# Visual-Behavior/aloception-oss

Measured on AMD Instinct MI355X. Metric: frames/sec (whole node) DeformableDETR-R50 inference, higher is better.
Workload: dtype bf16; 1 GPU; DeformableDETR-R50 inference bf16, batch 8 synthetic 1333x800 frames per GPU, random-init weights; launch=hip-graph replay + eager inference(), per_gpu_batch=8, global_batch=8, parallelism=batch-sharded x1, no collective

## Files before the change

aloception-oss_amd/csrc/gemm.hip:

```cpp
#include "common.hpp"

namespace alo {
namespace {

constexpr int kRows = 64;
constexpr int kOutStride = 64 * 2 + 16;

typedef __attribute__((ext_vector_type(8))) __bf16 bf16x8_t;

__device__ __forceinline__ bf16x8_t as_bf16x8(const u32x4& v) {
    union { u32x4 u; bf16x8_t b; } x;
    x.u = v;
    return x.b;
}

struct GemmDims {
    long M;
    int N;
    int tiles;
    int S;
    int gs, gWo, gHoWo, gW, gHW;
};

template <typename D>
__device__ __forceinline__ long gather_row(const D& dm, long row) {
    if (dm.gs <= 1) return row;
    const long n = row / dm.gHoWo;
    const int rem = (int)(row - n * dm.gHoWo);
    const int yo = rem / dm.gWo, xo = rem - yo * dm.gWo;
    return n * dm.gHW + (long)(yo * dm.gs) * dm.gW + xo * dm.gs;
}

template <int kK, bool RELU, bool HAS_RES, bool HM>
__global__ void __launch_bounds__(256, 2)
linear_shortk_kernel(const bf16_t* __restrict__ X, const bf16_t* __restrict__ W, const bf16_t* __restrict__ bias,
                     const bf16_t* __restrict__ R, bf16_t* __restrict__ Y, const GemmDims dm) {
    constexpr int kRowBytes = kK * 2 + 16;
    constexpr int kSteps = kK / 16;
    constexpr int kPieces = kK / 8;
    constexpr int kLoads = kRows * kPieces / 256;
    static_assert(kRows * kPieces % 256 == 0, "the tile loader gives every thread the same number of pieces");
    extern __shared__ __attribute__((aligned(16))) unsigned char smem[];
    unsigned char* const xbuf = smem;
    const int tid = threadIdx.x, wave = tid >> 6, lane = tid & 63;
    unsigned char* obuf = smem + kRows * kRowBytes + wave * (kRows * kOutStride);

    const int col0 = blockIdx.y * 256 + wave * 64;
    const bool has_cols = col0 < dm.N;
    const int nl = lane & 31, kg = lane >> 5;

    u32x4 wreg[2][kSteps];
    float* const bias_tab = reinterpret_cast<float*>(smem + kRows * kRowBytes + 4 * (kRows * kOutStride)) + wave * 64;
    if (has_cols) {
#pragma unroll
        for (int t = 0; t < 2; ++t) {
            const bf16_t* wr = W + (size_t)(col0 + 32 * t + nl) * kK + 8 * kg;
#pragma unroll
            for (int s = 0; s < kSteps; ++s) wreg[t][s] = *reinterpret_cast<const u32x4*>(wr + 16 * s);
        }
        const int r = lane & 15, t = (lane >> 4) & 1, k2 = lane >> 5;
        bias_tab[lane] = bias != nullptr ? bf16_to_f32(bias[col0 + 32 * t + (r & 3) + 8 * (r >> 2) + 4 * k2].bits) : 0.f;
    }

    auto fetch = [&](int tile, u32x4 (&r)[kLoads]) {
#pragma unroll
        for (int j = 0; j < kLoads; ++j) {
            const int p = tid + 256 * j;
            long row = (long)tile * kRows + p / kPieces;
            row = gather_row(dm, row < dm.M ? row : dm.M - 1);
            r[j] = *reinterpret_cast<const u32x4*>(X + row * kK + (p % kPieces) * 8);
        }
    };
    auto park = [&](const u32x4 (&r)[kLoads]) {
#pragma unroll
        for (int j = 0; j < kLoads; ++j) {
            const int p = tid + 256 * j;
            *reinterpret_cast<u32x4*>(xbuf + (p / kPieces) * kRowBytes + (p % kPieces) * 16) = r[j];
        }
    };

    int tile = blockIdx.x;
    if (tile >= dm.tiles) return;
    u32x4 stage[kLoads];
    fetch(tile, stage);

    for (;;) {
        park(stage);
        __syncthreads();
        const int next = tile + gridDim.x;
        const bool more = next < dm.tiles;
        if (more) fetch(next, stage);

        if (has_cols) {
#pragma unroll
            for (int half = 0; half < kRows / 32; ++half) {
                f32x16 acc[2];
#pragma unroll
                for (int t = 0; t < 2; ++t)
#pragma unroll
                    for (int q = 0; q < 4; ++q) {
                        const f32x4 b4 = *reinterpret_cast<const f32x4*>(bias_tab + (kg * 2 + t) * 16 + 4 * q);
#pragma unroll
                        for (int i = 0; i < 4; ++i) acc[t][4 * q + i] = b4[i];
                    }
#pragma unroll
                for (int s = 0; s < kSteps; ++s) {
                    const u32x4 a = *reinterpret_cast<const u32x4*>(xbuf + (32 * half + nl) * kRowBytes + (16 * s + 8 * kg) * 2);
                    acc[0] = __builtin_amdgcn_mfma_f32_32x32x16_bf16(as_bf16x8(wreg[0][s]), as_bf16x8(a), acc[0], 0, 0, 0);
                    acc[1] = __builtin_amdgcn_mfma_f32_32x32x16_bf16(as_bf16x8(wreg[1][s]), as_bf16x8(a), acc[1], 0, 0, 0);
                }
#pragma unroll
                for (int t = 0; t < 2; ++t)
#pragma unroll
                    for (int q = 0; q < 4; ++q) {
                        float v0 = acc[t][4 * q], v1 = acc[t][4 * q + 1], v2 = acc[t][4 * q + 2], v3 = acc[t][4 * q + 3];
                        if (RELU && !HAS_RES) { v0 = relu_keep_nan(v0); v1 = relu_keep_nan(v1); v2 = relu_keep_nan(v2); v3 = relu_keep_nan(v3); }
                        *reinterpret_cast<u32x2*>(obuf + (32 * half + nl) * kOutStride + (32 * t + 8 * q + 4 * kg) * 2) =
                            u32x2{pack_bf16x2(v0, v1), pack_bf16x2(v2, v3)};
                    }
            }
            __builtin_amdgcn_fence(__ATOMIC_RELEASE, "wavefront");
            __builtin_amdgcn_wave_barrier();
            __builtin_amdgcn_fence(__ATOMIC_ACQUIRE, "wavefront");
            if constexpr (HM) {
                const unsigned char* mask = reinterpret_cast<const unsigned char*>(R);
                const int heads = dm.N / 32;
#pragma unroll
                for (int hh = 0; hh < 2; ++hh) {
#pragma unroll
                    for (int pass = 0; pass < kRows / 16; ++pass) {
                        const int row = pass * 16 + (lane >> 2);
                        const long grow = (long)tile * kRows + row;
                        if (grow < dm.M) {
                            u32x4 v = *reinterpret_cast<const u32x4*>(obuf + row * kOutStride + hh * 64 + (lane & 3) * 16);
                            if (mask != nullptr && mask[grow]) v = u32x4{0u, 0u, 0u, 0u};
                            const long nb = grow / dm.S, sp = grow - nb * dm.S;
                            const int head = col0 / 32 + hh;
                            *reinterpret_cast<u32x4*>(Y + ((nb * heads + head) * dm.S + sp) * 32 + (lane & 3) * 8) = v;
                        }
                    }
                }
            } else
#pragma unroll
            for (int pass = 0; pass < kRows / 8; ++pass) {
                const int row = pass * 8 + (lane >> 3);
                const long grow = (long)tile * kRows + row;
                u32x4 v = *reinterpret_cast<const u32x4*>(obuf + row * kOutStride + (lane & 7) * 16);
                if (grow < dm.M) {
                    if constexpr (HAS_RES) {
                        const u32x4 rv = *reinterpret_cast<const u32x4*>(R + grow * dm.N + col0 + (lane & 7) * 8);
                        const unsigned a4[4] = {v.x, v.y, v.z, v.w}, r4[4] = {rv.x, rv.y, rv.z, rv.w};
                        unsigned o4[4];
#pragma unroll
                        for (int i = 0; i < 4; ++i) {
                            float lo = __uint_as_float(a4[i] << 16) + __uint_as_float(r4[i] << 16);
                            float hi = __uint_as_float(a4[i] & 0xffff0000u) + __uint_as_float(r4[i] & 0xffff0000u);
                            if (RELU) { lo = relu_keep_nan(lo); hi = relu_keep_nan(hi); }
                            o4[i] = pack_bf16x2(lo, hi);
                        }
                        v = u32x4{o4[0], o4[1], o4[2], o4[3]};
                    }
                    *reinterpret_cast<u32x4*>(Y + grow * dm.N + col0 + (lane & 7) * 8) = v;
                }
            }
        }
        if (!more) break;
        __syncthreads();
        tile = next;
    }
}

}
}

using namespace alo;

namespace {
template <int K, bool RELU, bool HAS_RES, bool HM = false>
int launch_shortk(const void* x, const void* weight, const void* bias, const void* residual, void* y, long M, int N,
                  hipStream_t stream, int S = 0, const int* gather = nullptr) {
    GemmDims dm;
    dm.M = M; dm.N = N; dm.tiles = (int)((M + kRows - 1) / kRows); dm.S = S;
    dm.gs = gather ? gather[0] : 1;
    dm.gWo = gather ? gather[2] : 1; dm.gHoWo = gather ? gather[1] * gather[2] : 1;
    dm.gW = gather ? gather[4] : 1; dm.gHW = gather ? gather[3] * gather[4] : 1;
    const size_t lds = kRows * (K * 2 + 16) + 4 * kRows * kOutStride + 4 * 64 * sizeof(float);
    const int cols = (N + 255) / 256;
    int gx = 512 / cols;
    if (gx > dm.tiles) gx = dm.tiles;
    if (gx < 1) gx = 1;
    void* args[] = {&x, &weight, &bias, &residual, &y, &dm};
    static unsigned long long attr_done = 0;
    (void)ensure_dynamic_lds(reinterpret_cast<const void*>(linear_shortk_kernel<K, RELU, HAS_RES, HM>), (int)lds, &attr_done);
    hipError_t e = hipLaunchKernel(reinterpret_cast<const void*>(linear_shortk_kernel<K, RELU, HAS_RES, HM>), dim3(gx, cols), dim3(256), args,
                                   lds, stream);
    if (e != hipSuccess) return fail(ALO_ERR_LAUNCH, "alo_linear_shortk: %s", hipGetErrorString(e));
    return check_launch("alo_linear_shortk");
}
}

extern "C" int alo_linear_shortk(const void* x, const void* weight, const void* bias, const void* residual, void* y, long M,
                                 int N, int K, int relu, int dtype, void* stream) {
    ALO_REQUIRE(x && weight && y, ALO_ERR_INVALID_ARGUMENT, "alo_linear_shortk: null pointer argument");
    ALO_REQUIRE(M > 0 && N > 0 && N % 64 == 0, ALO_ERR_INVALID_ARGUMENT,
                "alo_linear_shortk: M must be positive and N a positive multiple of 64 (M=%ld N=%d)", M, N);
    ALO_REQUIRE(K == 64 || K == 128 || K == 256, ALO_ERR_UNSUPPORTED, "alo_linear_shortk: K must be 64, 128 or 256, got %d", K);
    ALO_REQUIRE(dtype == ALO_BF16, ALO_ERR_UNSUPPORTED, "alo_linear_shortk: bf16 only (dtype %d)", dtype);
    ALO_REQUIRE((((uintptr_t)x | (uintptr_t)weight | (uintptr_t)y | (uintptr_t)residual) & 15) == 0, ALO_ERR_INVALID_ARGUMENT,
                "alo_linear_shortk: pointers must be 16-byte aligned");
    hipStream_t st = static_cast<hipStream_t>(stream);
#define ALO_GEMM_CASE(KK)                                                                                       \
    if (K == KK) {                                                                                               \
        if (residual) return relu ? launch_shortk<KK, true, true>(x, weight, bias, residual, y, M, N, st)       \
                                  : launch_shortk<KK, false, true>(x, weight, bias, residual, y, M, N, st);     \
        return relu ? launch_shortk<KK, true, false>(x, weight, bias, residual, y, M, N, st)                    \
                    : launch_shortk<KK, false, false>(x, weight, bias, residual, y, M, N, st);                  \
    }
    ALO_GEMM_CASE(64) ALO_GEMM_CASE(128) ALO_GEMM_CASE(256)
#undef ALO_GEMM_CASE
    return ALO_ERR_UNSUPPORTED;
}

extern "C" int alo_internal_shortk_gather(const void* x, const void* weight, const void* bias, const void* residual, void* y,
                                          long M, int N, int K, int relu, const int* gather, void* stream) {
    hipStream_t st = static_cast<hipStream_t>(stream);
#define ALO_GEMM_CASE(KK)                                                                                                  \
    if (K == KK) {                                                                                                          \
        if (residual) return relu ? launch_shortk<KK, true, true>(x, weight, bias, residual, y, M, N, st, 0, gather)       \
                                  : launch_shortk<KK, false, true>(x, weight, bias, residual, y, M, N, st, 0, gather);     \
        return relu ? launch_shortk<KK, true, false>(x, weight, bias, residual, y, M, N, st, 0, gather)                    \
                    : launch_shortk<KK, false, false>(x, weight, bias, residual, y, M, N, st, 0, gather);                  \
    }
    ALO_GEMM_CASE(64) ALO_GEMM_CASE(128) ALO_GEMM_CASE(256)
#undef ALO_GEMM_CASE
    return fail(ALO_ERR_UNSUPPORTED, "alo_conv1x1_nhwc: the resident-weight kernel needs Cin in (64, 128, 256), got %d", K);
}

namespace alo {
namespace {

constexpr int kFfnRows = 64;
constexpr int kFfnStride = 256 * 2 + 16;

struct FfnDims {
    long M;
    int F;
    int tiles;
};

__global__ void __launch_bounds__(256, 2)
ffn256_kernel(const bf16_t* __restrict__ X, const bf16_t* __restrict__ W1, const bf16_t* __restrict__ B1,
              const bf16_t* __restrict__ W2, const bf16_t* __restrict__ B2, bf16_t* __restrict__ Y, const FfnDims dm) {
    extern __shared__ __attribute__((aligned(16))) unsigned char smem[];
    unsigned char* const xs = smem;
    unsigned char* const hs = smem + kFfnRows * kFfnStride;
    const int tid = threadIdx.x, wave = tid >> 6, lane = tid & 63;
    const int nl = lane & 31, kg = lane >> 5;
    const int F = dm.F;

    float* const b1s = reinterpret_cast<float*>(smem + 2 * kFfnRows * kFfnStride);
    float* const b2s = b1s + F;
    for (int i = tid; i < F; i += 256) b1s[i] = B1 ? bf16_to_f32(B1[i].bits) : 0.f;
    b2s[tid] = B2 ? bf16_to_f32(B2[tid].bits) : 0.f;

    constexpr int KB = 2;
    constexpr int NBATCH = 16 / KB;
    auto load_batch = [&](u32x4 (&buf)[2][KB], const bf16_t* frag0, size_t tile_stride, int batch) {
#pragma unroll
        for (int t = 0; t < 2; ++t)
#pragma unroll
            for (int j = 0; j < KB; ++j)
                buf[t][j] = *reinterpret_cast<const u32x4*>(frag0 + t * tile_stride + (size_t)(KB * batch + j) * 512);
        __builtin_amdgcn_sched_barrier(0);
    };
    auto mma_batch = [&](f32x16 (&acc)[2][2], const unsigned char* a_lds, const u32x4 (&buf)[2][KB], int batch) {
        u32x4 af[2][KB];
#pragma unroll
        for (int j = 0; j < KB; ++j) {
            const int s = KB * batch + j;
            af[0][j] = *reinterpret_cast<const u32x4*>(a_lds + nl * kFfnStride + (16 * s + 8 * kg) * 2);
            af[1][j] = *reinterpret_cast<const u32x4*>(a_lds + (32 + nl) * kFfnStride + (16 * s + 8 * kg) * 2);
        }
#pragma unroll
        for (int j = 0; j < KB; ++j) {
            const u32x4 a0 = af[0][j], a1 = af[1][j];
            acc[0][0] = __builtin_amdgcn_mfma_f32_32x32x16_bf16(as_bf16x8(buf[0][j]), as_bf16x8(a0), acc[0][0], 0, 0, 0);
            acc[0][1] = __builtin_amdgcn_mfma_f32_32x32x16_bf16(as_bf16x8(buf[1][j]), as_bf16x8(a0), acc[0][1], 0, 0, 0);
            acc[1][0] = __builtin_amdgcn_mfma_f32_32x32x16_bf16(as_bf16x8(buf[0][j]), as_bf16x8(a1), acc[1][0], 0, 0, 0);
            acc[1][1] = __builtin_amdgcn_mfma_f32_32x32x16_bf16(as_bf16x8(buf[1][j]), as_bf16x8(a1), acc[1][1], 0, 0, 0);
        }
        __builtin_amdgcn_sched_barrier(0);
    };
    const int fs = F / 16;
    auto w1_frag = [&](int r0) { return W1 + ((size_t)((r0 + 64 * wave) / 32) * 16 * 64 + lane) * 8; };
    auto w2_frag = [&](int r0) { return W2 + (((size_t)(2 * wave) * fs + r0 / 16) * 64 + lane) * 8; };

    for (int tile = blockIdx.x; tile < dm.tiles; tile += gridDim.x) {
        {
            u32x4 xv[8];
#pragma unroll
            for (int j = 0; j < 8; ++j) {
                const int p = tid + 256 * j;
                long row = (long)tile * kFfnRows + (p >> 5);
                row = row < dm.M ? row : dm.M - 1;
                xv[j] = *reinterpret_cast<const u32x4*>(X + row * 256 + (p & 31) * 8);
            }
#pragma unroll
            for (int j = 0; j < 8; ++j) {
                const int p = tid + 256 * j;
                *reinterpret_cast<u32x4*>(xs + (p >> 5) * kFfnStride + (p & 31) * 16) = xv[j];
            }
        }
        u32x4 bufa[2][KB], bufb[2][KB];
        load_batch(bufa, w1_frag(0), (size_t)16 * 512, 0);
        __syncthreads();

        f32x16 acc2[2][2];
#pragma unroll
        for (int a = 0; a < 2; ++a)
#pragma unroll
            for (int t = 0; t < 2; ++t)
#pragma unroll
                for (int i = 0; i < 16; ++i) acc2[a][t][i] = 0.f;

        for (int r0 = 0; r0 < F; r0 += 256) {
            f32x16 acc1[2][2];
#pragma unroll
            for (int a = 0; a < 2; ++a)
#pragma unroll
                for (int t = 0; t < 2; ++t)
#pragma unroll
                    for (int i = 0; i < 16; ++i) acc1[a][t][i] = 0.f;
            const bf16_t* w1p = w1_frag(r0);
            const bf16_t* w2p = w2_frag(r0);
#pragma unroll
            for (int bt = 0; bt < NBATCH; bt += 2) {
                load_batch(bufb, w1p, (size_t)16 * 512, bt + 1);
                mma_batch(acc1, xs, bufa, bt);
                if (bt + 2 < NBATCH) load_batch(bufa, w1p, (size_t)16 * 512, bt + 2);
                else load_batch(bufa, w2p, (size_t)fs * 512, 0);
                mma_batch(acc1, xs, bufb, bt + 1);
            }
#pragma unroll
            for (int t = 0; t < 2; ++t)
#pragma unroll
                for (int q = 0; q < 4; ++q) {
                    const int col = 64 * wave + 32 * t + 8 * q + 4 * kg;
                    const f32x4 bb = *reinterpret_cast<const f32x4*>(b1s + r0 + col);
#pragma unroll
                    for (int a = 0; a < 2; ++a) {
                        const float v0 = relu_keep_nan(acc1[a][t][4 * q] + bb[0]), v1 = relu_keep_nan(acc1[a][t][4 * q + 1] + bb[1]);
                        const float v2 = relu_keep_nan(acc1[a][t][4 * q + 2] + bb[2]), v3 = relu_keep_nan(acc1[a][t][4 * q + 3] + bb[3]);
                        *reinterpret_cast<u32x2*>(hs + (32 * a + nl) * kFfnStride + col * 2) = u32x2{pack_bf16x2(v0, v1), pack_bf16x2(v2, v3)};
                    }
                }
            __syncthreads();

#pragma unroll
            for (int bt = 0; bt < NBATCH; bt += 2) {
                load_batch(bufb, w2p, (size_t)fs * 512, bt + 1);
                mma_batch(acc2, hs, bufa, bt);
                if (bt + 2 < NBATCH) load_batch(bufa, w2p, (size_t)fs * 512, bt + 2);
                else if (r0 + 256 < F) load_batch(bufa, w1_frag(r0 + 256), (size_t)16 * 512, 0);
                mma_batch(acc2, hs, bufb, bt + 1);
            }
            __syncthreads();
        }

#pragma unroll
        for (int t = 0; t < 2; ++t)
#pragma unroll
            for (int q = 0; q < 4; ++q) {
                const int col = 64 * wave + 32 * t + 8 * q + 4 * kg;
                const f32x4 bb = *reinterpret_cast<const f32x4*>(b2s + col);
#pragma unroll
                for (int a = 0; a < 2; ++a)
                    *reinterpret_cast<u32x2*>(hs + (32 * a + nl) * kFfnStride + col * 2) =
                        u32x2{pack_bf16x2(acc2[a][t][4 * q] + bb[0], acc2[a][t][4 * q + 1] + bb[1]),
                              pack_bf16x2(acc2[a][t][4 * q + 2] + bb[2], acc2[a][t][4 * q + 3] + bb[3])};
            }
        __syncthreads();
#pragma unroll
        for (int j = 0; j < 8; ++j) {
            const int p = tid + 256 * j;
            const long row = (long)tile * kFfnRows + (p >> 5);
            if (row < dm.M)
                *reinterpret_cast<u32x4*>(Y + row * 256 + (p & 31) * 8) =
                    *reinterpret_cast<const u32x4*>(hs + (p >> 5) * kFfnStride + (p & 31) * 16);
        }
        __syncthreads();
    }
}

}
}

namespace alo {
namespace {
__global__ void __launch_bounds__(256)
pack_mfma_b_kernel(const bf16_t* __restrict__ W, bf16_t* __restrict__ P, int N, int K) {
    const long total = (long)N * K / 8;
    for (long i = (long)blockIdx.x * 256 + threadIdx.x; i < total; i += (long)gridDim.x * 256) {
        const int lane = (int)(i % 64);
        const long frag = i / 64;
        const int s = (int)(frag % (K / 16)), t = (int)(frag / (K / 16));
        const int n = 32 * t + (lane & 31), k = 16 * s + 8 * (lane >> 5);
        *reinterpret_cast<u32x4*>(P + i * 8) = *reinterpret_cast<const u32x4*>(W + (size_t)n * K + k);
    }
}
}
}

extern "C" int alo_pack_mfma_b(const void* w, void* packed, int N, int K, int dtype, void* stream) {
    ALO_REQUIRE(w && packed, ALO_ERR_INVALID_ARGUMENT, "alo_pack_mfma_b: null pointer argument");
    ALO_REQUIRE(N > 0 && K > 0 && N % 32 == 0 && K % 16 == 0, ALO_ERR_INVALID_ARGUMENT,
                "alo_pack_mfma_b: N must be a multiple of 32 and K a multiple of 16 (N=%d K=%d)", N, K);
    ALO_REQUIRE(dtype == ALO_BF16, ALO_ERR_UNSUPPORTED, "alo_pack_mfma_b: bf16 only (dtype %d)", dtype);
    long total = (long)N * K / 8;
    unsigned blocks = (unsigned)((total + 255) / 256 > 4096 ? 4096 : (total + 255) / 256);
    void* args[] = {&w, &packed, &N, &K};
    hipError_t e = hipLaunchKernel(reinterpret_cast<const void*>(pack_mfma_b_kernel), dim3(blocks), dim3(256), args, 0,
                                   static_cast<hipStream_t>(stream));
    if (e != hipSuccess) return fail(ALO_ERR_LAUNCH, "alo_pack_mfma_b: %s", hipGetErrorString(e));
    return check_launch("alo_pack_mfma_b");
}

extern "C" int alo_ffn256(const void* x, const void* w1, const void* b1, const void* w2, const void* b2, void* y, long M,
                          int F, int dtype, void* stream) {
    ALO_REQUIRE(x && w1 && w2 && y, ALO_ERR_INVALID_ARGUMENT, "alo_ffn256: null pointer argument");
    ALO_REQUIRE(M > 0 && F > 0 && F % 256 == 0, ALO_ERR_INVALID_ARGUMENT,
                "alo_ffn256: M must be positive and the hidden width a positive multiple of 256 (M=%ld F=%d)", M, F);
    ALO_REQUIRE(dtype == ALO_BF16, ALO_ERR_UNSUPPORTED, "alo_ffn256: bf16 only (dtype %d)", dtype);
    ALO_REQUIRE((((uintptr_t)x | (uintptr_t)w1 | (uintptr_t)w2 | (uintptr_t)y) & 15) == 0, ALO_ERR_INVALID_ARGUMENT,
                "alo_ffn256: pointers must be 16-byte aligned");
    FfnDims dm;
    dm.M = M; dm.F = F; dm.tiles = (int)((M + kFfnRows - 1) / kFfnRows);
    const size_t lds = 2 * kFfnRows * kFfnStride + ((size_t)F + 256) * sizeof(float);
    int gx = dm.tiles < 512 ? dm.tiles : 512;
    void* args[] = {&x, &w1, &b1, &w2, &b2, &y, &dm};
    if (lds > 160 * 1024) return fail(ALO_ERR_UNSUPPORTED, "alo_ffn256: hidden width %d needs %zu bytes of LDS", F, lds);
    {
        static int limit_set[64] = {0};
        int dev = 0;
        (void)hipGetDevice(&dev);
        if ((int)lds > __atomic_load_n(&limit_set[dev & 63], __ATOMIC_ACQUIRE)) {
            if (hipFuncSetAttribute(reinterpret_cast<const void*>(ffn256_kernel), hipFuncAttributeMaxDynamicSharedMemorySize, (int)lds) == hipSuccess)
                __atomic_store_n(&limit_set[dev & 63], (int)lds, __ATOMIC_RELEASE);
        }
    }
    hipError_t e = hipLaunchKernel(reinterpret_cast<const void*>(ffn256_kernel), dim3(gx), dim3(256), args, lds,
                                   static_cast<hipStream_t>(stream));
    if (e != hipSuccess) return fail(ALO_ERR_LAUNCH, "alo_ffn256: %s", hipGetErrorString(e));
    return check_launch("alo_ffn256");
}

extern "C" int alo_value_proj_head_major(const void* x, const void* weight, const void* bias, const void* padding_mask,
                                         void* value_hm, int batch, int S, int heads, int K, int dtype, void* stream) {
    ALO_REQUIRE(x && weight && value_hm, ALO_ERR_INVALID_ARGUMENT, "alo_value_proj_head_major: null pointer argument");
    ALO_REQUIRE(batch > 0 && S > 0 && heads > 0 && heads % 2 == 0, ALO_ERR_INVALID_ARGUMENT,
                "alo_value_proj_head_major: batch, S must be positive and the head count even (batch=%d S=%d heads=%d)", batch, S,
                heads);
    ALO_REQUIRE(K == 64 || K == 128 || K == 256, ALO_ERR_UNSUPPORTED, "alo_value_proj_head_major: K must be 64, 128 or 256, got %d", K);
    ALO_REQUIRE(dtype == ALO_BF16, ALO_ERR_UNSUPPORTED, "alo_value_proj_head_major: bf16 only (dtype %d)", dtype);
    ALO_REQUIRE((((uintptr_t)x | (uintptr_t)weight | (uintptr_t)value_hm) & 15) == 0, ALO_ERR_INVALID_ARGUMENT,
                "alo_value_proj_head_major: pointers must be 16-byte aligned");
    hipStream_t st = static_cast<hipStream_t>(stream);
    const long M = (long)batch * S;
    const int N = heads * 32;
    if (K == 64) return launch_shortk<64, false, false, true>(x, weight, bias, padding_mask, value_hm, M, N, st, S);
    if (K == 128) return launch_shortk<128, false, false, true>(x, weight, bias, padding_mask, value_hm, M, N, st, S);
    return launch_shortk<256, false, false, true>(x, weight, bias, padding_mask, value_hm, M, N, st, S);
}
```

Measured before the change: 840.7 frames/s.

## Add small-M fused FFN kernel using 32-row tiles and 512 threads

```diff
diff --git a/aloception-oss_amd/csrc/gemm.hip b/aloception-oss_amd/csrc/gemm.hip
--- a/aloception-oss_amd/csrc/gemm.hip
+++ b/aloception-oss_amd/csrc/gemm.hip
@@ -392,6 +392,151 @@
     }
 }
 
+constexpr int kShRows = 32;
+constexpr int kShThreads = 512;
+constexpr int kShStride = kFfnStride;
+
+struct FfnShDims {
+    long M;
+    int F;
+    long units;
+};
+
+template <int RT, int KB>
+__device__ __forceinline__ void ffn_sh_tile(const bf16_t* __restrict__ X, const bf16_t* __restrict__ W1, const bf16_t* __restrict__ W2,
+                                            bf16_t* __restrict__ Y, const long row0, const long M, const int F,
+                                            unsigned char* xs, unsigned char* hs, const float* b1s, const float* b2s, const int tid,
+                                            const int wave, const int lane) {
+    constexpr int NBATCH = 16 / KB;
+    static_assert(NBATCH % 2 == 0, "batches are consumed in pairs");
+    const int nl = lane & 31, kg = lane >> 5;
+
+    {
+        u32x4 xv[2 * RT];
+#pragma unroll
+        for (int j = 0; j < 2 * RT; ++j) {
+            const int p = tid + kShThreads * j;
+            long row = row0 + (p >> 5);
+            row = row < M ? row : M - 1;
+            xv[j] = *reinterpret_cast<const u32x4*>(X + row * 256 + (p & 31) * 8);
+        }
+#pragma unroll
+        for (int j = 0; j < 2 * RT; ++j) {
+            const int p = tid + kShThreads * j;
+            *reinterpret_cast<u32x4*>(xs + (p >> 5) * kShStride + (p & 31) * 16) = xv[j];
+        }
+    }
+
+    auto load_batch = [&](u32x4 (&buf)[KB], const bf16_t* frag0, int batch) {
+#pragma unroll
+        for (int j = 0; j < KB; ++j) buf[j] = *reinterpret_cast<const u32x4*>(frag0 + (size_t)(KB * batch + j) * 512);
+        __builtin_amdgcn_sched_barrier(0);
+    };
+    auto mma_batch = [&](f32x16 (&acc)[RT], const unsigned char* a_lds, const u32x4 (&buf)[KB], int batch) {
+        u32x4 af[RT][KB];
+#pragma unroll
+        for (int j = 0; j < KB; ++j)
+#pragma unroll
+            for (int rt = 0; rt < RT; ++rt)
+                af[rt][j] = *reinterpret_cast<const u32x4*>(a_lds + (32 * rt + nl) * kShStride + (16 * (KB * batch + j) + 8 * kg) * 2);
+#pragma unroll
+        for (int j = 0; j < KB; ++j)
+#pragma unroll
+            for (int rt = 0; rt < RT; ++rt)
+                acc[rt] = __builtin_amdgcn_mfma_f32_32x32x16_bf16(as_bf16x8(buf[j]), as_bf16x8(af[rt][j]), acc[rt], 0, 0, 0);
+        __builtin_amdgcn_sched_barrier(0);
+    };
+    const int fs = F / 16;
+    auto w1_frag = [&](int r0) { return W1 + ((size_t)((r0 + 32 * wave) / 32) * 16 * 64 + lane) * 8; };
+    auto w2_frag = [&](int r0) { return W2 + (((size_t)wave * fs + r0 / 16) * 64 + lane) * 8; };
+
+    u32x4 bufa[KB], bufb[KB];
+    load_batch(bufa, w1_frag(0), 0);
+    __syncthreads();
+
+    f32x16 acc2[RT];
+#pragma unroll
+    for (int rt = 0; rt < RT; ++rt)
+#pragma unroll
+        for (int i = 0; i < 16; ++i) acc2[rt][i] = 0.f;
+
+    for (int r0 = 0; r0 < F; r0 += 256) {
+        f32x16 acc1[RT];
+#pragma unroll
+        for (int rt = 0; rt < RT; ++rt)
+#pragma unroll
+            for (int i = 0; i < 16; ++i) acc1[rt][i] = 0.f;
+        const bf16_t* w1p = w1_frag(r0);
+        const bf16_t* w2p = w2_frag(r0);
+#pragma unroll
+        for (int bt = 0; bt < NBATCH; bt += 2) {
+            load_batch(bufb, w1p, bt + 1);
+            mma_batch(acc1, xs, bufa, bt);
+            if (bt + 2 < NBATCH) load_batch(bufa, w1p, bt + 2);
+            else load_batch(bufa, w2p, 0);
+            mma_batch(acc1, xs, bufb, bt + 1);
+        }
+#pragma unroll
+        for (int q = 0; q < 4; ++q) {
+            const int col = 32 * wave + 8 * q + 4 * kg;
+            const f32x4 bb = *reinterpret_cast<const f32x4*>(b1s + r0 + col);
+#pragma unroll
+            for (int rt = 0; rt < RT; ++rt) {
+                const float v0 = relu_keep_nan(acc1[rt][4 * q] + bb[0]), v1 = relu_keep_nan(acc1[rt][4 * q + 1] + bb[1]);
+                const float v2 = relu_keep_nan(acc1[rt][4 * q + 2] + bb[2]), v3 = relu_keep_nan(acc1[rt][4 * q + 3] + bb[3]);
+                *reinterpret_cast<u32x2*>(hs + (32 * rt + nl) * kShStride + col * 2) = u32x2{pack_bf16x2(v0, v1), pack_bf16x2(v2, v3)};
+            }
+        }
+        __syncthreads();
+
+#pragma unroll
+        for (int bt = 0; bt < NBATCH; bt += 2) {
+            load_batch(bufb, w2p, bt + 1);
+            mma_batch(acc2, hs, bufa, bt);
+            if (bt + 2 < NBATCH) load_batch(bufa, w2p, bt + 2);
+            else if (r0 + 256 < F) load_batch(bufa, w1_frag(r0 + 256), 0);
+            mma_batch(acc2, hs, bufb, bt + 1);
+        }
+        __syncthreads();
+    }
+
+#pragma unroll
+    for (int q = 0; q < 4; ++q) {
+        const int col = 32 * wave + 8 * q + 4 * kg;
+        const f32x4 bb = *reinterpret_cast<const f32x4*>(b2s + col);
+#pragma unroll
+        for (int rt = 0; rt < RT; ++rt)
+            *reinterpret_cast<u32x2*>(hs + (32 * rt + nl) * kShStride + col * 2) =
+                u32x2{pack_bf16x2(acc2[rt][4 * q] + bb[0], acc2[rt][4 * q + 1] + bb[1]),
+                      pack_bf16x2(acc2[rt][4 * q + 2] + bb[2], acc2[rt][4 * q + 3] + bb[3])};
+    }
+    __syncthreads();
+#pragma unroll
+    for (int j = 0; j < 2 * RT; ++j) {
+        const int p = tid + kShThreads * j;
+        const long row = row0 + (p >> 5);
+        if (row < M)
+            *reinterpret_cast<u32x4*>(Y + row * 256 + (p & 31) * 8) = *reinterpret_cast<const u32x4*>(hs + (p >> 5) * kShStride + (p & 31) * 16);
+    }
+    __syncthreads();
+}
+
+__global__ void __launch_bounds__(kShThreads, 1)
+ffn256_small_kernel(const bf16_t* __restrict__ X, const bf16_t* __restrict__ W1, const bf16_t* __restrict__ B1,
+                     const bf16_t* __restrict__ W2, const bf16_t* __restrict__ B2, bf16_t* __restrict__ Y, const FfnShDims dm) {
+    extern __shared__ __attribute__((aligned(16))) unsigned char smem[];
+    unsigned char* const xs = smem;
+    unsigned char* const hs = smem + kShRows * kShStride;
+    float* const b1s = reinterpret_cast<float*>(smem + 2 * kShRows * kShStride);
+    float* const b2s = b1s + dm.F;
+    const int tid = threadIdx.x, wave = tid >> 6, lane = tid & 63;
+    for (int i = tid; i < dm.F; i += kShThreads) b1s[i] = B1 ? bf16_to_f32(B1[i].bits) : 0.f;
+    if (tid < 256) b2s[tid] = B2 ? bf16_to_f32(B2[tid].bits) : 0.f;
+
+    const long u0 = dm.units * blockIdx.x / gridDim.x, u1 = dm.units * (blockIdx.x + 1) / gridDim.x;
+    for (long u = u0; u < u1; ++u) ffn_sh_tile<1, 8>(X, W1, W2, Y, u * 32, dm.M, dm.F, xs, hs, b1s, b2s, tid, wave, lane);
+}
+
 }
 }
 
@@ -433,6 +578,28 @@
     ALO_REQUIRE(dtype == ALO_BF16, ALO_ERR_UNSUPPORTED, "alo_ffn256: bf16 only (dtype %d)", dtype);
     ALO_REQUIRE((((uintptr_t)x | (uintptr_t)w1 | (uintptr_t)w2 | (uintptr_t)y) & 15) == 0, ALO_ERR_INVALID_ARGUMENT,
                 "alo_ffn256: pointers must be 16-byte aligned");
+    hipStream_t st = static_cast<hipStream_t>(stream);
+    static int cus[64] = {0};
+    int dev = 0;
+    (void)hipGetDevice(&dev);
+    int ncu = __atomic_load_n(&cus[dev & 63], __ATOMIC_ACQUIRE);
+    if (ncu <= 0) {
+        if (hipDeviceGetAttribute(&ncu, hipDeviceAttributeMultiprocessorCount, dev) != hipSuccess || ncu <= 0) ncu = 256;
+        __atomic_store_n(&cus[dev & 63], ncu, __ATOMIC_RELEASE);
+    }
+    const long units = (M + 31) / 32;
+    const size_t lds_sm = 2 * kShRows * kShStride + ((size_t)F + 256) * sizeof(float);
+    if (units <= ncu && lds_sm <= 160 * 1024) {
+        static unsigned long long attr_done = 0;
+        (void)ensure_dynamic_lds(reinterpret_cast<const void*>(ffn256_small_kernel), 160 * 1024, &attr_done);
+        FfnShDims sd;
+        sd.M = M; sd.F = F; sd.units = units;
+        void* args[] = {&x, &w1, &b1, &w2, &b2, &y, &sd};
+        hipError_t e = hipLaunchKernel(reinterpret_cast<const void*>(ffn256_small_kernel), dim3((unsigned)units), dim3(kShThreads), args,
+                                       lds_sm, st);
+        if (e != hipSuccess) return fail(ALO_ERR_LAUNCH, "alo_ffn256: %s", hipGetErrorString(e));
+        return check_launch("alo_ffn256");
+    }
     FfnDims dm;
     dm.M = M; dm.F = F; dm.tiles = (int)((M + kFfnRows - 1) / kFfnRows);
     const size_t lds = 2 * kFfnRows * kFfnStride + ((size_t)F + 256) * sizeof(float);
@@ -441,15 +608,12 @@
     if (lds > 160 * 1024) return fail(ALO_ERR_UNSUPPORTED, "alo_ffn256: hidden width %d needs %zu bytes of LDS", F, lds);
     {
         static int limit_set[64] = {0};
-        int dev = 0;
-        (void)hipGetDevice(&dev);
         if ((int)lds > __atomic_load_n(&limit_set[dev & 63], __ATOMIC_ACQUIRE)) {
             if (hipFuncSetAttribute(reinterpret_cast<const void*>(ffn256_kernel), hipFuncAttributeMaxDynamicSharedMemorySize, (int)lds) == hipSuccess)
                 __atomic_store_n(&limit_set[dev & 63], (int)lds, __ATOMIC_RELEASE);
         }
     }
-    hipError_t e = hipLaunchKernel(reinterpret_cast<const void*>(ffn256_kernel), dim3(gx), dim3(256), args, lds,
-                                   static_cast<hipStream_t>(stream));
+    hipError_t e = hipLaunchKernel(reinterpret_cast<const void*>(ffn256_kernel), dim3(gx), dim3(256), args, lds, st);
     if (e != hipSuccess) return fail(ALO_ERR_LAUNCH, "alo_ffn256: %s", hipGetErrorString(e));
     return check_launch("alo_ffn256");
 }
```

Result: no change. 850.0 frames/s, median of 6 (+1.1%).
